# viswavi/speech-anonymization

Hardware: AMD Instinct MI355X
Metric: audio frames/sec (node), ConvAE+gender-adv train step (higher is better)
Workload: dtype bf16x3; 1 GPU; ConvAE recon0.1+sex0.9 adversarial train step (L1 recon + NLL), shape M: 32 utt/GPU x 161120 samples (T=1008 frames), Fbank x2 + norm + fwd + bwd + clip + Adam + Noam; batch_per_gpu=32, frames_per_utt=1008, parallelism=dp1

## Files before the change

### speech-anonymization_amd/csrc/sa_common.h

```cpp
#pragma once
#include <hip/hip_runtime.h>
#include <stdint.h>
#include "../../include/sa_hip.h"

typedef __bf16 bf16_t;
typedef __bf16 bf16x8 __attribute__((ext_vector_type(8)));
typedef float f32x16 __attribute__((ext_vector_type(16)));
typedef float f32x4 __attribute__((ext_vector_type(4)));

#define SA_WAVE 64


template <typename T> struct Tr;

template <> struct Tr<float> {
  static constexpr int VEC = 4;
  static constexpr int KS = 2;
  typedef float Frag;
  __device__ static inline void unpack(const uint4& u, float* f) {
    f[0] = __uint_as_float(u.x); f[1] = __uint_as_float(u.y);
    f[2] = __uint_as_float(u.z); f[3] = __uint_as_float(u.w);
  }
  __device__ static inline uint4 pack(const float* f) {
    return make_uint4(__float_as_uint(f[0]), __float_as_uint(f[1]),
                      __float_as_uint(f[2]), __float_as_uint(f[3]));
  }
  __device__ static inline float to_f(float v) { return v; }
  __device__ static inline float from_f(float v) { return v; }
  __device__ static inline f32x16 mfma(Frag a, Frag b, f32x16 c) {
    return __builtin_amdgcn_mfma_f32_32x32x2f32(a, b, c, 0, 0, 0);
  }
};

__device__ static inline uint32_t sa_pack_bf16x2(float lo, float hi) {
  union { bf16_t b[2]; uint32_t u; } cv;
  cv.b[0] = (bf16_t)lo; cv.b[1] = (bf16_t)hi;
  return cv.u;
}

template <> struct Tr<bf16_t> {
  static constexpr int VEC = 8;
  static constexpr int KS = 16;
  typedef bf16x8 Frag;
  __device__ static inline void unpack(const uint4& u, float* f) {
    f[0] = __uint_as_float(u.x << 16); f[1] = __uint_as_float(u.x & 0xffff0000u);
    f[2] = __uint_as_float(u.y << 16); f[3] = __uint_as_float(u.y & 0xffff0000u);
    f[4] = __uint_as_float(u.z << 16); f[5] = __uint_as_float(u.z & 0xffff0000u);
    f[6] = __uint_as_float(u.w << 16); f[7] = __uint_as_float(u.w & 0xffff0000u);
  }
  __device__ static inline uint4 pack(const float* f) {
    return make_uint4(sa_pack_bf16x2(f[0], f[1]), sa_pack_bf16x2(f[2], f[3]),
                      sa_pack_bf16x2(f[4], f[5]), sa_pack_bf16x2(f[6], f[7]));
  }
  __device__ static inline float to_f(bf16_t v) { return (float)v; }
  __device__ static inline bf16_t from_f(float v) { return (bf16_t)v; }
  __device__ static inline f32x16 mfma(Frag a, Frag b, f32x16 c) {
    return __builtin_amdgcn_mfma_f32_32x32x16_bf16(a, b, c, 0, 0, 0);
  }
};

__device__ static inline float sa_swish(float v) { return v * __builtin_amdgcn_rcpf(1.0f + __expf(-v)); }
__device__ static inline float sa_swish_grad(float v) {
  const float s = __builtin_amdgcn_rcpf(1.0f + __builtin_amdgcn_exp2f(v * -1.4426950408889634f));
  const float t = 1.0f - s;
  const float u = fmaf(v, t, 1.0f);
  return s * u;
}

__device__ static inline int sa_acc_row(int reg, int lane) {
  return (reg & 3) + 8 * (reg >> 2) + 4 * (lane >> 5);
}

__device__ static inline float sa_wave_sum(float v) {
#pragma unroll
  for (int o = 32; o > 0; o >>= 1) v += __shfl_xor(v, o, 64);
  return v;
}
__device__ static inline double sa_wave_sum_d(double v) {
#pragma unroll
  for (int o = 32; o > 0; o >>= 1) v += __shfl_xor(v, o, 64);
  return v;
}
__device__ static inline float sa_wave_max(float v) {
#pragma unroll
  for (int o = 32; o > 0; o >>= 1) v = fmaxf(v, __shfl_xor(v, o, 64));
  return v;
}

static inline int sa_div_up(int a, int b) { return (a + b - 1) / b; }

struct bf16x3_t {};
struct bf16x1f_t {};

struct fp8_t {};
typedef long fp8x8;

template <typename T> struct Pol;
template <> struct Pol<float> {
  typedef float store_t; typedef float lds_t; typedef float Frag;
  static constexpr int NPL = 1, VEC = 4, KS = 2, PAD = 1;
};
template <> struct Pol<bf16_t> {
  typedef bf16_t store_t; typedef bf16_t lds_t; typedef bf16x8 Frag;
  static constexpr int NPL = 1, VEC = 8, KS = 16, PAD = 8;
};
template <> struct Pol<bf16x1f_t> {
  typedef float store_t; typedef bf16_t lds_t; typedef bf16x8 Frag;
  static constexpr int NPL = 1, VEC = 4, KS = 16, PAD = 8;
};
template <> struct Pol<bf16x3_t> {
  typedef float store_t; typedef bf16_t lds_t; typedef bf16x8 Frag;
  static constexpr int NPL = 2, VEC = 4, KS = 16, PAD = 8;
};

template <> struct Pol<fp8_t> {
  typedef bf16_t store_t; typedef unsigned char lds_t; typedef fp8x8 Frag;
  static constexpr int NPL = 1, VEC = 8, KS = 16, PAD = 8;
};
template <> struct Tr<unsigned char> {
  __device__ static inline f32x16 mfma(fp8x8 a, fp8x8 b, f32x16 c) {
    return __builtin_amdgcn_mfma_f32_32x32x16_fp8_fp8(a, b, c, 0, 0, 0);
  }
};
__device__ static inline uint2 sa_pack_fp8x8(const float* f) {
  float c[8];
#pragma unroll
  for (int j = 0; j < 8; ++j) c[j] = __builtin_amdgcn_fmed3f(f[j], -448.0f, 448.0f);
  int lo = 0, hi = 0;
  lo = __builtin_amdgcn_cvt_pk_fp8_f32(c[0], c[1], lo, false);
  lo = __builtin_amdgcn_cvt_pk_fp8_f32(c[2], c[3], lo, true);
  hi = __builtin_amdgcn_cvt_pk_fp8_f32(c[4], c[5], hi, false);
  hi = __builtin_amdgcn_cvt_pk_fp8_f32(c[6], c[7], hi, true);
  return make_uint2((unsigned)lo, (unsigned)hi);
}

__device__ static inline uint2 sa_pack_bf16x4(const float* f) {
  return make_uint2(sa_pack_bf16x2(f[0], f[1]), sa_pack_bf16x2(f[2], f[3]));
}
__device__ static inline void sa_split4(const float* f, uint2& hi, uint2& lo) {
  float h[4], l[4];
#pragma unroll
  for (int j = 0; j < 4; ++j) {
    const bf16_t hb = (bf16_t)f[j];
    h[j] = (float)hb;
    l[j] = f[j] - h[j];
  }
  hi = sa_pack_bf16x4(h);
  lo = sa_pack_bf16x4(l);
}
```

### speech-anonymization_amd/csrc/sa_head.hip

```cpp
#include "sa_common.h"

template <typename T>
__global__ __launch_bounds__(256) void sa_pool_fwd_kernel(const T* __restrict__ r,
                                                          const float* __restrict__ sc,
                                                          const float* __restrict__ sh,
                                                          float* __restrict__ part, int L,
                                                          int nseg) {
  constexpr int C = 128, VEC = Tr<T>::VEC, CH = C / VEC, RPB = 256 / CH, NG = 128 / RPB;
  __shared__ float tile[RPB][C][2];
  const int tid = threadIdx.x, b = blockIdx.y, grp = blockIdx.x % NG, seg = blockIdx.x / NG;
  const int c = tid % CH, rl = tid / CH, lm = grp * RPB + rl;
  float s[VEC], t[VEC], sum[VEC], sq[VEC];
#pragma unroll
  for (int j = 0; j < VEC; ++j) { s[j] = sc[c * VEC + j]; t[j] = sh[c * VEC + j]; sum[j] = 0.f; sq[j] = 0.f; }
  const int nk = (L + 127) / 128, per = (nk + nseg - 1) / nseg;
  const int kbeg = seg * per, kend = (kbeg + per < nk) ? kbeg + per : nk;
  const T* rb = r + (size_t)b * L * C + c * VEC;
  for (int k0 = kbeg; k0 < kend; k0 += 4) {
    uint4 raw[4];
#pragma unroll
    for (int i = 0; i < 4; ++i) {
      const int l = lm + 128 * (k0 + i);
      raw[i] = make_uint4(0, 0, 0, 0);
      if (k0 + i < kend && l < L) raw[i] = *reinterpret_cast<const uint4*>(rb + (size_t)l * C);
    }
#pragma unroll
    for (int i = 0; i < 4; ++i) {
      const int l = lm + 128 * (k0 + i);
      if (k0 + i < kend && l < L) {
        float f[VEC];
        Tr<T>::unpack(raw[i], f);
#pragma unroll
        for (int j = 0; j < VEC; ++j) {
          const float v = fmaf(f[j], s[j], t[j]);
          sum[j] += v; sq[j] = fmaf(v, v, sq[j]);
        }
      }
    }
  }
#pragma unroll
  for (int j = 0; j < VEC; ++j) { tile[rl][c * VEC + j][0] = sum[j]; tile[rl][c * VEC + j][1] = sq[j]; }
  __syncthreads();
  float* dst = part + ((size_t)b * nseg + seg) * C * 128 * 2;
  for (int e = tid; e < RPB * C * 2; e += 256) {
    const int cc = e / (RPB * 2), w = e % (RPB * 2);
    dst[((size_t)cc * 128 + grp * RPB) * 2 + w] = tile[w >> 1][cc][w & 1];
  }
}

__global__ __launch_bounds__(1024) void sa_pool_gather_kernel(const float* __restrict__ part, int nseg,
                                                              int L, double* __restrict__ sums) {
  __shared__ double grp[7][128][2];
  const int tid = threadIdx.x, b = blockIdx.x, j = tid & 127, h = tid >> 7, Lm = L % 128;
  double s = 0.0, q = 0.0;
  for (int seg = 0; seg < nseg; ++seg) {
    const float2* p = reinterpret_cast<const float2*>(part) + ((size_t)b * nseg + seg) * 128 * 128;
#pragma unroll 16
    for (int c = h * 16; c < h * 16 + 16; ++c) {
      const float2 v = p[(size_t)c * 128 + ((j - c * Lm) & 127)];
      s += v.x; q += v.y;
    }
  }
  if (h > 0) { grp[h - 1][j][0] = s; grp[h - 1][j][1] = q; }
  __syncthreads();
  if (h == 0) {
#pragma unroll
    for (int g = 0; g < 7; ++g) { s += grp[g][j][0]; q += grp[g][j][1]; }
    sums[((size_t)b * 128 + j) * 2 + 0] = s;
    sums[((size_t)b * 128 + j) * 2 + 1] = q;
  }
}

extern "C" int sa_pool_nseg(int B) {
  int n = 2048 / (B * 16);
  return n < 1 ? 1 : (n > 8 ? 8 : n);
}

extern "C" int sa_pool_fwd(int dtype, const void* r, const float* scale, const float* shift,
                           float* part, int B, int L, int nseg, void* stream) {
  if (!r || !scale || !shift || !part || B <= 0 || L <= 1 || nseg < 1) return -22;
  hipStream_t st = reinterpret_cast<hipStream_t>(stream);
  if (dtype == SA_BF16)
    hipLaunchKernelGGL(sa_pool_fwd_kernel<bf16_t>, dim3(8 * nseg, B), dim3(256), 0, st,
                       reinterpret_cast<const bf16_t*>(r), scale, shift, part, L, nseg);
  else
    hipLaunchKernelGGL(sa_pool_fwd_kernel<float>, dim3(16 * nseg, B), dim3(256), 0, st,
                       reinterpret_cast<const float*>(r), scale, shift, part, L, nseg);
  hipError_t e = hipGetLastError();
  return e == hipSuccess ? 0 : -(int)e;
}

extern "C" int sa_pool_gather(const float* part, int B, int nseg, int L, double* sums, void* stream) {
  if (!part || !sums || B <= 0 || nseg < 1) return -22;
  hipLaunchKernelGGL(sa_pool_gather_kernel, dim3(B), dim3(1024), 0,
                     reinterpret_cast<hipStream_t>(stream), part, nseg, L, sums);
  hipError_t e = hipGetLastError();
  return e == hipSuccess ? 0 : -(int)e;
}

__global__ void sa_pool_fin_kernel(const double* __restrict__ sums, int B, int n,
                                   const float* __restrict__ noise, float eps, float* pooled,
                                   float* mean, float* stdraw) {
  const int i = blockIdx.x * blockDim.x + threadIdx.x;
  if (i >= B * 128) return;
  const int b = i / 128, j = i % 128;
  const double S = sums[2 * i], Q = sums[2 * i + 1];
  const double m = S / n;
  double var = (Q - S * m) / (n - 1);
  if (var < 0.0) var = 0.0;
  const float sd = (float)sqrt(var);
  mean[i] = (float)m; stdraw[i] = sd;
  float mo = (float)m;
  if (noise) mo += eps * ((1.0f - 9.0f) * noise[i] + 9.0f);
  pooled[(size_t)b * 256 + j] = mo;
  pooled[(size_t)b * 256 + 128 + j] = sd + eps;
}

extern "C" int sa_pool_fin(const double* sums, int B, int n, const float* noise, float eps,
                           float* pooled, float* mean, float* stdraw, void* stream) {
  if (!sums || !pooled || !mean || !stdraw || n < 2) return -22;
  hipLaunchKernelGGL(sa_pool_fin_kernel, dim3(sa_div_up(B * 128, 256)), dim3(256), 0,
                     reinterpret_cast<hipStream_t>(stream), sums, B, n, noise, eps, pooled, mean,
                     stdraw);
  hipError_t e = hipGetLastError();
  return e == hipSuccess ? 0 : -(int)e;
}

template <typename T>
__global__ __launch_bounds__(256) void sa_pool_bwd_kernel(const T* __restrict__ r,
                                                          const float* __restrict__ sc,
                                                          const float* __restrict__ sh,
                                                          const float* __restrict__ dpooled,
                                                          const float* __restrict__ mean,
                                                          const float* __restrict__ stdraw,
                                                          T* __restrict__ g, int L,
                                                          const float* __restrict__ bn_mean,
                                                          const float* __restrict__ bn_rstd,
                                                          float* __restrict__ stats) {
  constexpr int C = 128, VEC = Tr<T>::VEC, CH = C / VEC, RPP = 256 / CH;
  __shared__ float ka[128], kb[128];
  __shared__ float red[RPP][C][2];
  const int tid = threadIdx.x, b = blockIdx.y, l0 = blockIdx.x * SA_WAVE * 4;
  if (tid < 128) {
    const float dm = dpooled[(size_t)b * 256 + tid], ds = dpooled[(size_t)b * 256 + 128 + tid];
    const float sd = stdraw[(size_t)b * 128 + tid], m = mean[(size_t)b * 128 + tid];
    const float inv = sd > 0.0f ? 1.0f / ((float)(L - 1) * sd) : 0.0f;
    kb[tid] = ds * inv;
    ka[tid] = dm / (float)L - ds * inv * m;
  }
  __syncthreads();
  const int c = tid % CH, r0 = tid / CH;
  float s[VEC], t[VEC];
  int jb[VEC];
#pragma unroll
  for (int j = 0; j < VEC; ++j) {
    s[j] = sc[c * VEC + j]; t[j] = sh[c * VEC + j];
    jb[j] = (int)(((long long)(c * VEC + j) * L) % 128);
  }
  float bm[VEC], br[VEC], s1[VEC], s2[VEC];
#pragma unroll
  for (int j = 0; j < VEC; ++j) {
    bm[j] = stats ? bn_mean[c * VEC + j] : 0.0f;
    br[j] = stats ? bn_rstd[c * VEC + j] : 0.0f;
    s1[j] = 0.0f; s2[j] = 0.0f;
  }
  for (int rr = r0; rr < 256; rr += RPP) {
    const int l = l0 + rr;
    if (l >= L) break;
    float f[VEC], x[VEC];
    Tr<T>::unpack(*reinterpret_cast<const uint4*>(r + ((size_t)b * L + l) * C + c * VEC), x);
#pragma unroll
    for (int j = 0; j < VEC; ++j) {
      const int col = (jb[j] + l) % 128;
      f[j] = fmaf(kb[col], fmaf(x[j], s[j], t[j]), ka[col]);
    }
    const uint4 u = Tr<T>::pack(f);
    *reinterpret_cast<uint4*>(g + ((size_t)b * L + l) * C + c * VEC) = u;
    if (stats) {
      Tr<T>::unpack(u, f);
#pragma unroll
      for (int j = 0; j < VEC; ++j) {
        s1[j] += f[j];
        s2[j] = fmaf(f[j], (x[j] - bm[j]) * br[j], s2[j]);
      }
    }
  }
  if (stats) {
#pragma unroll
    for (int j = 0; j < VEC; ++j) { red[r0][c * VEC + j][0] = s1[j]; red[r0][c * VEC + j][1] = s2[j]; }
    __syncthreads();
    if (tid < C) {
      float a0 = 0.0f, a1 = 0.0f;
#pragma unroll
      for (int q = 0; q < RPP; ++q) { a0 += red[q][tid][0]; a1 += red[q][tid][1]; }
      float* dst = stats + (((size_t)b * gridDim.x + blockIdx.x) * C + tid) * 2;
      dst[0] = a0; dst[1] = a1;
    }
  }
}

extern "C" int sa_pool_bwd(int dtype, const void* r, const float* scale, const float* shift,
                           const float* dpooled, const float* mean, const float* stdraw, void* g,
                           int B, int L, const float* bn_mean, const float* bn_rstd, float* stats,
                           void* stream) {
  if (!r || !scale || !shift || !dpooled || !mean || !stdraw || !g || L < 2) return -22;
  if (stats && (!bn_mean || !bn_rstd)) return -22;
  hipStream_t st = reinterpret_cast<hipStream_t>(stream);
  dim3 grid(sa_div_up(L, 256), B);
  if (dtype == SA_BF16)
    hipLaunchKernelGGL(sa_pool_bwd_kernel<bf16_t>, grid, dim3(256), 0, st,
                       reinterpret_cast<const bf16_t*>(r), scale, shift, dpooled, mean, stdraw,
                       reinterpret_cast<bf16_t*>(g), L, bn_mean, bn_rstd, stats);
  else
    hipLaunchKernelGGL(sa_pool_bwd_kernel<float>, grid, dim3(256), 0, st,
                       reinterpret_cast<const float*>(r), scale, shift, dpooled, mean, stdraw,
                       reinterpret_cast<float*>(g), L, bn_mean, bn_rstd, stats);
  hipError_t e = hipGetLastError();
  return e == hipSuccess ? 0 : -(int)e;
}

__global__ __launch_bounds__(256) void sa_dense_kernel(const float* __restrict__ X, int lda,
                                                       const float* __restrict__ ps,
                                                       const float* __restrict__ pt,
                                                       const float* __restrict__ W, int sbk, int sbn,
                                                       const float* __restrict__ bias, float* __restrict__ Y,
                                                       int ldy, int M, int N, int K, int relu) {
  __shared__ float part[4][16][64];
  const int lane = threadIdx.x & 63, wave = threadIdx.x >> 6, n0 = blockIdx.x * 32, m0 = blockIdx.y * 32;
  const int m = m0 + (lane & 31), n = n0 + (lane & 31), kh = lane >> 5;
  f32x16 acc;
#pragma unroll
  for (int i = 0; i < 16; ++i) acc[i] = 0.0f;
  for (int k0 = wave * 16; k0 < K; k0 += 64) {
    float av[8], bv[8];
#pragma unroll
    for (int u = 0; u < 8; ++u) {
      const int k = k0 + 2 * u + kh;
      av[u] = 0.0f; bv[u] = 0.0f;
      if (k < K) {
        if (m < M) {
          av[u] = X[(size_t)m * lda + k];
          if (ps) av[u] = fmaf(av[u], ps[k], pt[k]);
        }
        if (n < N) bv[u] = W[(size_t)k * sbk + (size_t)n * sbn];
      }
    }
#pragma unroll
    for (int u = 0; u < 8; ++u)
      if (k0 + 2 * u < K) acc = __builtin_amdgcn_mfma_f32_32x32x2f32(av[u], bv[u], acc, 0, 0, 0);
  }
#pragma unroll
  for (int i = 0; i < 16; ++i) part[wave][i][lane] = acc[i];
  __syncthreads();
  if (wave == 0 && n < N) {
    const float bb = bias ? bias[n] : 0.0f;
#pragma unroll
    for (int i = 0; i < 16; ++i) {
      const int mr = m0 + sa_acc_row(i, lane);
      if (mr < M) {
        float v = ((part[0][i][lane] + part[1][i][lane]) + part[2][i][lane]) + part[3][i][lane] + bb;
        if (relu) v = fmaxf(v, 0.0f);
        Y[(size_t)mr * ldy + n] = v;
      }
    }
  }
}

extern "C" int sa_dense(const float* X, int lda, const float* ps, const float* pt, const float* W,
                        int sbk, int sbn, const float* bias, float* Y, int ldy, int M, int N, int K,
                        int relu, void* stream) {
  if (!X || !W || !Y || M <= 0 || N <= 0 || K <= 0) return -22;
  dim3 grid(sa_div_up(N, 32), sa_div_up(M, 32));
  hipLaunchKernelGGL(sa_dense_kernel, grid, dim3(256), 0, reinterpret_cast<hipStream_t>(stream), X,
                     lda, ps, pt, W, sbk, sbn, bias, Y, ldy, M, N, K, relu);
  hipError_t e = hipGetLastError();
  return e == hipSuccess ? 0 : -(int)e;
}

__global__ void sa_colsums_kernel(const float* __restrict__ X, const float* __restrict__ H,
                                  const float* __restrict__ hm, const float* __restrict__ hr,
                                  int M, int N, double* sums, float* __restrict__ out0,
                                  float* __restrict__ out1) {
  const int n = blockIdx.x * blockDim.x + threadIdx.x;
  if (n >= N) return;
  double s = 0.0, q = 0.0;
#pragma unroll 8
  for (int m = 0; m < M; ++m) {
    const float x = X[(size_t)m * N + n];
    float h = H ? H[(size_t)m * N + n] : x;
    if (hm) h = (h - hm[n]) * hr[n];
    s += x; q += (double)x * h;
  }
  sums[2 * n] = s; sums[2 * n + 1] = q;
  if (out0) out0[n] = (float)s;
  if (out1) out1[n] = (float)q;
}

extern "C" int sa_colsums(const float* X, const float* H, const float* hmean, const float* hrstd,
                          int M, int N, double* sums, float* out0, float* out1, void* stream) {
  if (!X || !sums) return -22;
  hipLaunchKernelGGL(sa_colsums_kernel, dim3(sa_div_up(N, 64)), dim3(64), 0,
                     reinterpret_cast<hipStream_t>(stream), X, H, hmean, hrstd, M, N, sums, out0,
                     out1);
  hipError_t e = hipGetLastError();
  return e == hipSuccess ? 0 : -(int)e;
}

__global__ void sa_bn2d_bwd_kernel(const float* __restrict__ G, const float* __restrict__ H,
                                   const double* __restrict__ sums, double count,
                                   const float* __restrict__ gamma, const float* __restrict__ mean,
                                   const float* __restrict__ rstd, int relu_mask, int M, int N,
                                   float* dH, const double* __restrict__ count_dev) {
  const int i = blockIdx.x * blockDim.x + threadIdx.x;
  if (i >= M * N) return;
  if (count_dev) count = *count_dev;
  const int n = i % N;
  const float hh = (H[i] - mean[n]) * rstd[n];
  float v = gamma[n] * rstd[n] * (G[i] - (float)(sums[2 * n] / count) - hh * (float)(sums[2 * n + 1] / count));
  if (relu_mask && !(H[i] > 0.0f)) v = 0.0f;
  dH[i] = v;
}

extern "C" int sa_bn2d_bwd(const float* G, const float* H, const double* sums, double count,
                           const float* gamma, const float* mean, const float* rstd, int relu_mask,
                           int M, int N, float* dH, const double* count_dev, void* stream) {
  if (!G || !H || !sums || !gamma || !mean || !rstd || !dH) return -22;
  hipLaunchKernelGGL(sa_bn2d_bwd_kernel, dim3(sa_div_up(M * N, 256)), dim3(256), 0,
                     reinterpret_cast<hipStream_t>(stream), G, H, sums, count, gamma, mean, rstd,
                     relu_mask, M, N, dH, count_dev);
  hipError_t e = hipGetLastError();
  return e == hipSuccess ? 0 : -(int)e;
}

__global__ void sa_dense_wgrad_kernel(const float* __restrict__ dY, const float* __restrict__ X,
                                      const float* __restrict__ ps, const float* __restrict__ pt,
                                      int M, int N, int K, float* dW) {
  const int i = blockIdx.x * blockDim.x + threadIdx.x;
  if (i >= N * K) return;
  const int n = i / K, k = i % K;
  float s = 0.0f;
#pragma unroll 8
  for (int m = 0; m < M; ++m) {
    float x = X[(size_t)m * K + k];
    if (ps) x = fmaf(x, ps[k], pt[k]);
    s = fmaf(dY[(size_t)m * N + n], x, s);
  }
  dW[i] = s;
}

extern "C" int sa_dense_wgrad(const float* dY, const float* X, const float* ps, const float* pt,
                              int M, int N, int K, float* dW, void* stream) {
  if (!dY || !X || !dW) return -22;
  hipLaunchKernelGGL(sa_dense_wgrad_kernel, dim3(sa_div_up(N * K, 256)), dim3(256), 0,
                     reinterpret_cast<hipStream_t>(stream), dY, X, ps, pt, M, N, K, dW);
  hipError_t e = hipGetLastError();
  return e == hipSuccess ? 0 : -(int)e;
}

__global__ void sa_log_softmax_kernel(const float* __restrict__ X, float* __restrict__ Y, int M, int N) {
  const int m = blockIdx.x * blockDim.x + threadIdx.x;
  if (m >= M) return;
  float mx = -INFINITY;
  for (int n = 0; n < N; ++n) mx = fmaxf(mx, X[(size_t)m * N + n]);
  float s = 0.0f;
  for (int n = 0; n < N; ++n) s += expf(X[(size_t)m * N + n] - mx);
  const float lse = mx + logf(s);
  for (int n = 0; n < N; ++n) Y[(size_t)m * N + n] = X[(size_t)m * N + n] - lse;
}
__global__ void sa_log_softmax_bwd_kernel(const float* __restrict__ dY, const float* __restrict__ Y,
                                          float* __restrict__ dX, int M, int N) {
  const int m = blockIdx.x * blockDim.x + threadIdx.x;
  if (m >= M) return;
  float s = 0.0f;
  for (int n = 0; n < N; ++n) s += dY[(size_t)m * N + n];
  for (int n = 0; n < N; ++n) dX[(size_t)m * N + n] = dY[(size_t)m * N + n] - expf(Y[(size_t)m * N + n]) * s;
}
extern "C" int sa_log_softmax(const float* X, float* Y, int M, int N, void* stream) {
  if (!X || !Y) return -22;
  hipLaunchKernelGGL(sa_log_softmax_kernel, dim3(sa_div_up(M, 64)), dim3(64), 0,
                     reinterpret_cast<hipStream_t>(stream), X, Y, M, N);
  hipError_t e = hipGetLastError();
  return e == hipSuccess ? 0 : -(int)e;
}
extern "C" int sa_log_softmax_bwd(const float* dY, const float* Y, float* dX, int M, int N, void* stream) {
  if (!dY || !Y || !dX) return -22;
  hipLaunchKernelGGL(sa_log_softmax_bwd_kernel, dim3(sa_div_up(M, 64)), dim3(64), 0,
                     reinterpret_cast<hipStream_t>(stream), dY, Y, dX, M, N);
  hipError_t e = hipGetLastError();
  return e == hipSuccess ? 0 : -(int)e;
}
// ... 138 lines not shown
```

### speech-anonymization_amd/csrc/sa_small.hip

```cpp
#include "sa_common.h"

#define SA_K15 15
#define SA_C32 32

template <typename T>
__global__ __launch_bounds__(256) void sa_conv1toC_kernel(const float* __restrict__ x,
                                                          const float* __restrict__ w,
                                                          const float* __restrict__ bias,
                                                          T* __restrict__ y, int L, int flip,
                                                          float* __restrict__ stats, int ntiles,
                                                          const T* __restrict__ ep_x,
                                                          const float* __restrict__ ep_s1,
                                                          const float* __restrict__ ep_t1,
                                                          const float* __restrict__ ep_mean,
                                                          const float* __restrict__ ep_rstd) {
  constexpr int VEC = Tr<T>::VEC, CH = SA_C32 / VEC, PPP = 256 / CH, TILE = 512;
  __shared__ float xs[TILE + SA_K15 - 1];
  __shared__ __attribute__((aligned(16))) float ws[SA_K15][SA_C32];
  __shared__ float red[PPP][SA_C32][2];
  const int tid = threadIdx.x, b = blockIdx.y, l0 = blockIdx.x * TILE;
  for (int i = tid; i < TILE + SA_K15 - 1; i += 256) {
    const int g = l0 + i - 7;
    xs[i] = (g >= 0 && g < L) ? x[(size_t)b * L + g] : 0.0f;
  }
  for (int i = tid; i < SA_K15 * SA_C32; i += 256) {
    const int k = i / SA_C32, c = i % SA_C32;
    ws[k][c] = w[c * SA_K15 + (flip ? SA_K15 - 1 - k : k)];
  }
  __syncthreads();
  const int c = tid % CH, p0 = tid / CH;
  float bv[VEC], ssum[VEC], ssq[VEC];
#pragma unroll
  for (int j = 0; j < VEC; ++j) { bv[j] = bias ? bias[c * VEC + j] : 0.0f; ssum[j] = 0.f; ssq[j] = 0.f; }
  float es[VEC], et[VEC], em[VEC], er[VEC];
#pragma unroll
  for (int j = 0; j < VEC; ++j) {
    const size_t bc = (size_t)b * SA_C32 + c * VEC + j;
    es[j] = ep_x ? ep_s1[bc] : 1.0f; et[j] = ep_x ? ep_t1[bc] : 0.0f;
    em[j] = ep_x ? ep_mean[bc] : 0.0f; er[j] = ep_x ? ep_rstd[bc] : 0.0f;
  }
  for (int p = p0; p < TILE; p += PPP) {
    const int l = l0 + p;
    if (l >= L) break;
    float acc[VEC];
#pragma unroll
    for (int j = 0; j < VEC; ++j) acc[j] = bv[j];
#pragma unroll
    for (int k = 0; k < SA_K15; ++k) {
      const float xv = xs[p + k];
#pragma unroll
      for (int j = 0; j < VEC; ++j) acc[j] = fmaf(xv, ws[k][c * VEC + j], acc[j]);
    }
    float xn[VEC];
    if (ep_x) {
      float xv[VEC];
      Tr<T>::unpack(*reinterpret_cast<const uint4*>(ep_x + ((size_t)b * L + l) * SA_C32 + c * VEC), xv);
#pragma unroll
      for (int j = 0; j < VEC; ++j) {
        acc[j] *= sa_swish_grad(fmaf(xv[j], es[j], et[j]));
        xn[j] = (xv[j] - em[j]) * er[j];
      }
    }
    const uint4 u = Tr<T>::pack(acc);
    *reinterpret_cast<uint4*>(y + ((size_t)b * L + l) * SA_C32 + c * VEC) = u;
    if (stats) {
      float f[VEC];
      Tr<T>::unpack(u, f);
#pragma unroll
      for (int j = 0; j < VEC; ++j) { ssum[j] += f[j]; ssq[j] = fmaf(f[j], ep_x ? xn[j] : f[j], ssq[j]); }
    }
  }
  if (stats) {
#pragma unroll
    for (int j = 0; j < VEC; ++j) { red[p0][c * VEC + j][0] = ssum[j]; red[p0][c * VEC + j][1] = ssq[j]; }
    __syncthreads();
    if (tid < SA_C32) {
      float s = 0.f, q = 0.f;
      for (int r = 0; r < PPP; ++r) { s += red[r][tid][0]; q += red[r][tid][1]; }
      float* d = stats + (((size_t)b * ntiles + blockIdx.x) * SA_C32 + tid) * 2;
      d[0] = s; d[1] = q;
    }
  }
}

extern "C" int sa_conv1toC_ntiles(int L) { return sa_div_up(L, 512); }

extern "C" int sa_conv1toC(int dtype, const float* x, const float* w, const float* bias, void* y,
                           int B, int L, int flip, float* stats, const void* ep_x, const float* ep_s1,
                           const float* ep_t1, const float* ep_mean, const float* ep_rstd,
                           void* stream) {
  if (!x || !w || !y || B <= 0 || L <= 0) return -22;
  if (ep_x && (!ep_s1 || !ep_t1 || !ep_mean || !ep_rstd)) return -22;
  hipStream_t st = reinterpret_cast<hipStream_t>(stream);
  const int nt = sa_div_up(L, 512);
  dim3 grid(nt, B);
  if (dtype == SA_BF16)
    hipLaunchKernelGGL(sa_conv1toC_kernel<bf16_t>, grid, dim3(256), 0, st, x, w, bias,
                       reinterpret_cast<bf16_t*>(y), L, flip, stats, nt,
                       reinterpret_cast<const bf16_t*>(ep_x), ep_s1, ep_t1, ep_mean, ep_rstd);
  else
    hipLaunchKernelGGL(sa_conv1toC_kernel<float>, grid, dim3(256), 0, st, x, w, bias,
                       reinterpret_cast<float*>(y), L, flip, stats, nt,
                       reinterpret_cast<const float*>(ep_x), ep_s1, ep_t1, ep_mean, ep_rstd);
  hipError_t e = hipGetLastError();
  return e == hipSuccess ? 0 : -(int)e;
}

template <typename T>
__global__ __launch_bounds__(256) void sa_convCto1_kernel(const T* __restrict__ x,
                                                          const float* __restrict__ w,
                                                          const float* __restrict__ bias,
                                                          float* __restrict__ y, int L,
                                                          const float* __restrict__ s1,
                                                          const float* __restrict__ t1, int swish,
                                                          int flip) {
  constexpr int VEC = Tr<T>::VEC, CH = SA_C32 / VEC, RPP = 256 / CH, TILE = 128, PITCH = 36;
  constexpr int NPOS = TILE + SA_K15 - 1, NBLK = (NPOS + 15) / 16, TP = 17;
  constexpr int NIT = (NBLK * 16 + RPP - 1) / RPP;
  __shared__ __attribute__((aligned(16))) float xs[NBLK * 16 * PITCH];
  __shared__ float tp[NBLK * 16 * TP];
  const int tid = threadIdx.x, lane = tid & 63, wave = tid >> 6, b = blockIdx.y, l0 = blockIdx.x * TILE;
  {
    const int c = tid % CH, r0 = tid / CH;
    float sc[VEC], sh[VEC];
#pragma unroll
    for (int j = 0; j < VEC; ++j) {
      sc[j] = s1 ? s1[(size_t)b * SA_C32 + c * VEC + j] : 1.0f;
      sh[j] = t1 ? t1[(size_t)b * SA_C32 + c * VEC + j] : 0.0f;
    }
    uint4 raw[NIT];
#pragma unroll
    for (int i = 0; i < NIT; ++i) {
      const int r = r0 + i * RPP, g = l0 + r - 7;
      raw[i] = make_uint4(0, 0, 0, 0);
      if (r < NPOS && g >= 0 && g < L)
        raw[i] = *reinterpret_cast<const uint4*>(x + ((size_t)b * L + g) * SA_C32 + c * VEC);
    }
#pragma unroll
    for (int i = 0; i < NIT; ++i) {
      const int r = r0 + i * RPP, g = l0 + r - 7;
      if (r < NBLK * 16) {
        float f[VEC];
        Tr<T>::unpack(raw[i], f);
        const bool valid = r < NPOS && g >= 0 && g < L;
#pragma unroll
        for (int j = 0; j < VEC; ++j) {
          float v = fmaf(f[j], sc[j], sh[j]);
          v = swish ? sa_swish(v) : v;
          xs[r * PITCH + c * VEC + j] = valid ? v : 0.0f;
        }
      }
    }
  }
  const int n = lane & 15, kq = lane >> 4;
  float wb[8];
#pragma unroll
  for (int ks = 0; ks < 8; ++ks)
    wb[ks] = n < SA_K15 ? w[(ks * 4 + kq) * SA_K15 + (flip ? SA_K15 - 1 - n : n)] : 0.0f;
  __syncthreads();
  for (int blk = wave; blk < NBLK; blk += 4) {
    f32x4 acc = {0.f, 0.f, 0.f, 0.f};
    const float* ap = xs + (blk * 16 + n) * PITCH + kq;
#pragma unroll
    for (int ks = 0; ks < 8; ++ks) acc = __builtin_amdgcn_mfma_f32_16x16x4f32(ap[ks * 4], wb[ks], acc, 0, 0, 0);
#pragma unroll
    for (int i = 0; i < 4; ++i) tp[(blk * 16 + 4 * kq + i) * TP + n] = acc[i];
  }
  __syncthreads();
  const int l = l0 + tid;
  if (tid < TILE && l < L) {
    float acc = bias ? bias[0] : 0.0f;
#pragma unroll
    for (int k = 0; k < SA_K15; ++k) acc += tp[(tid + k) * TP + k];
    y[(size_t)b * L + l] = acc;
  }
}

extern "C" int sa_convCto1(int dtype, const void* x, const float* w, const float* bias, float* y,
                           int B, int L, const float* s1, const float* t1, int swish, int flip,
                           void* stream) {
  if (!x || !w || !y || B <= 0 || L <= 0) return -22;
  hipStream_t st = reinterpret_cast<hipStream_t>(stream);
  dim3 grid(sa_div_up(L, 128), B);
  if (dtype == SA_BF16)
    hipLaunchKernelGGL(sa_convCto1_kernel<bf16_t>, grid, dim3(256), 0, st,
                       reinterpret_cast<const bf16_t*>(x), w, bias, y, L, s1, t1, swish, flip);
  else
    hipLaunchKernelGGL(sa_convCto1_kernel<float>, grid, dim3(256), 0, st,
                       reinterpret_cast<const float*>(x), w, bias, y, L, s1, t1, swish, flip);
  hipError_t e = hipGetLastError();
  return e == hipSuccess ? 0 : -(int)e;
}

template <typename T>
__global__ __launch_bounds__(256) void sa_wgrad1C_kernel(const float* __restrict__ u,
                                                         const T* __restrict__ v,
                                                         float* __restrict__ slabs, int L,
                                                         int chunk, int flip,
                                                         const float* __restrict__ s1,
                                                         const float* __restrict__ t1, int swish) {
  constexpr int VEC = Tr<T>::VEC, CH = SA_C32 / VEC, RPP = 256 / CH, TILE = 256, PITCH = 33;
  __shared__ float us[TILE + SA_K15 - 1 + 1];
  __shared__ float vs[TILE * PITCH];
  const int tid = threadIdx.x, lane = tid & 63, wave = tid >> 6, b = blockIdx.y;
  const int lbeg = blockIdx.x * chunk;
  int lend = lbeg + chunk; if (lend > L) lend = L;
  const int c = tid % CH, r0 = tid / CH;
  float sc[VEC], sh[VEC];
#pragma unroll
  for (int j = 0; j < VEC; ++j) {
    sc[j] = s1 ? s1[(size_t)b * SA_C32 + c * VEC + j] : 1.0f;
    sh[j] = t1 ? t1[(size_t)b * SA_C32 + c * VEC + j] : 0.0f;
  }
  const bool tr_on = (s1 != nullptr) || swish;
  const int m = lane & 15, j4 = lane >> 4;
  const bool mval = m < SA_K15;
  const int kk = mval ? (flip ? SA_K15 - 1 - m : m) : 0;
  const int qa = wave * 64 + 16 * j4;
  f32x4 acc0 = {0.f, 0.f, 0.f, 0.f}, acc1 = {0.f, 0.f, 0.f, 0.f};
  constexpr int NIT = TILE / RPP, NU = (TILE + SA_K15 - 1 + 255) / 256;
  uint4 raw[NIT];
  float rawu[NU];
  auto issue = [&](int l0) {
#pragma unroll
    for (int i = 0; i < NIT; ++i) {
      const int g = l0 + r0 + i * RPP;
      raw[i] = make_uint4(0, 0, 0, 0);
      if (g < lend) raw[i] = *reinterpret_cast<const uint4*>(v + ((size_t)b * L + g) * SA_C32 + c * VEC);
    }
#pragma unroll
    for (int i = 0; i < NU; ++i) {
      const int g = l0 + tid + i * 256 - 7;
      rawu[i] = (l0 < lend && tid + i * 256 < TILE + SA_K15 - 1 && g >= 0 && g < L) ? u[(size_t)b * L + g] : 0.0f;
    }
  };
  issue(lbeg);
  for (int l0 = lbeg; l0 < lend; l0 += TILE) {
#pragma unroll
    for (int i = 0; i < NU; ++i)
      if (tid + i * 256 < TILE + SA_K15 - 1) us[tid + i * 256] = rawu[i];
#pragma unroll
    for (int i = 0; i < NIT; ++i) {
      const int r = r0 + i * RPP, g = l0 + r;
      float f[VEC];
      Tr<T>::unpack(raw[i], f);
      if (tr_on && g < lend) {
#pragma unroll
        for (int j = 0; j < VEC; ++j) {
          float z = fmaf(f[j], sc[j], sh[j]);
          f[j] = swish ? sa_swish(z) : z;
        }
      }
#pragma unroll
      for (int j = 0; j < VEC; ++j) vs[r * PITCH + c * VEC + j] = f[j];
    }
    __syncthreads();
    issue(l0 + TILE);
#pragma unroll 4
    for (int t = 0; t < 16; ++t) {
      const int q = qa + t;
      const float av = mval ? us[q + kk] : 0.0f;
      const float b0 = vs[q * PITCH + m], b1 = vs[q * PITCH + 16 + m];
      acc0 = __builtin_amdgcn_mfma_f32_16x16x4f32(av, b0, acc0, 0, 0, 0);
      acc1 = __builtin_amdgcn_mfma_f32_16x16x4f32(av, b1, acc1, 0, 0, 0);
    }
    __syncthreads();
  }
  float* part = vs;
#pragma unroll
  for (int i = 0; i < 4; ++i) {
    part[(wave * 16 + 4 * j4 + i) * 32 + m] = acc0[i];
    part[(wave * 16 + 4 * j4 + i) * 32 + 16 + m] = acc1[i];
  }
  __syncthreads();
  for (int o = tid; o < SA_K15 * SA_C32; o += 256) {
    const int k = o / SA_C32, cc = o % SA_C32;
    const float sum = ((part[(0 * 16 + k) * 32 + cc] + part[(1 * 16 + k) * 32 + cc]) +
                       part[(2 * 16 + k) * 32 + cc]) + part[(3 * 16 + k) * 32 + cc];
    slabs[((size_t)b * gridDim.x + blockIdx.x) * (SA_C32 * SA_K15) + cc * SA_K15 + k] = sum;
  }
}

extern "C" int sa_wgrad1C_nchunk(int L, int chunk) { return sa_div_up(L, chunk); }

extern "C" int sa_wgrad1C(int dtype, const float* u, const void* v, float* slabs, int B, int L,
                          int chunk, int flip, const float* s1, const float* t1, int swish,
                          void* stream) {
  if (!u || !v || !slabs || B <= 0 || L <= 0 || chunk <= 0 || chunk % 256) return -22;
  hipStream_t st = reinterpret_cast<hipStream_t>(stream);
  dim3 grid(sa_div_up(L, chunk), B);
  if (dtype == SA_BF16)
    hipLaunchKernelGGL(sa_wgrad1C_kernel<bf16_t>, grid, dim3(256), 0, st, u,
                       reinterpret_cast<const bf16_t*>(v), slabs, L, chunk, flip, s1, t1, swish);
  else
    hipLaunchKernelGGL(sa_wgrad1C_kernel<float>, grid, dim3(256), 0, st, u,
                       reinterpret_cast<const float*>(v), slabs, L, chunk, flip, s1, t1, swish);
  hipError_t e = hipGetLastError();
  return e == hipSuccess ? 0 : -(int)e;
}

template <typename T>
__global__ __launch_bounds__(256, Tr<T>::VEC == 4 ? 3 : 2) void sa_bwd1C_kernel(const float* __restrict__ u,
                                                       const T* __restrict__ v,
                                                       const float* __restrict__ w,
                                                       T* __restrict__ gout, float* __restrict__ stats,
                                                       int ntiles, float* __restrict__ slabs, int L,
                                                       int chunk, int flip,
                                                       const float* __restrict__ s1,
                                                       const float* __restrict__ t1,
                                                       const float* __restrict__ mean,
                                                       const float* __restrict__ rstd) {
  constexpr int VEC = Tr<T>::VEC, CH = SA_C32 / VEC, RPP = 256 / CH, TILE = 256, PITCH = 33;
  __shared__ float us[TILE + SA_K15 - 1 + 1];
  __shared__ float vs[TILE * PITCH];
  __shared__ __attribute__((aligned(16))) float ws[SA_K15][SA_C32];
  __shared__ float red[RPP][SA_C32][2];
  __shared__ __attribute__((aligned(16))) float pv[4][SA_C32];
  const int tid = threadIdx.x, lane = tid & 63, wave = tid >> 6, b = blockIdx.y;
  const int lbeg = blockIdx.x * chunk;
  int lend = lbeg + chunk; if (lend > L) lend = L;
  const int c = tid % CH, r0 = tid / CH;
  float ssum[VEC], ssq[VEC];
#pragma unroll
  for (int j = 0; j < VEC; ++j) { ssum[j] = 0.f; ssq[j] = 0.f; }
  if (tid < 4 * SA_C32) {
    const float* src = tid < 32 ? s1 : tid < 64 ? t1 : tid < 96 ? mean : rstd;
    pv[tid >> 5][tid & 31] = src[(size_t)b * SA_C32 + (tid & 31)];
  }
  for (int i = tid; i < SA_K15 * SA_C32; i += 256) {
    const int k = i / SA_C32, cc = i % SA_C32;
    ws[k][cc] = w[cc * SA_K15 + (flip ? SA_K15 - 1 - k : k)];
  }
  const int m = lane & 15, j4 = lane >> 4;
  const bool mval = m < SA_K15;
  const int kk = mval ? (flip ? SA_K15 - 1 - m : m) : 0;
  const int qa = wave * 64 + 16 * j4;
  f32x4 acc0 = {0.f, 0.f, 0.f, 0.f}, acc1 = {0.f, 0.f, 0.f, 0.f};
  constexpr int NIT = TILE / RPP, NU = (TILE + SA_K15 - 1 + 255) / 256;
  uint4 raw[NIT];
  float rawu[NU];
  auto issue_v = [&](int l0, int i) {
    const int g = l0 + r0 + i * RPP;
    raw[i] = make_uint4(0, 0, 0, 0);
    if (g < lend) raw[i] = *reinterpret_cast<const uint4*>(v + ((size_t)b * L + g) * SA_C32 + c * VEC);
  };
  auto issue_u = [&](int l0) {
#pragma unroll
    for (int i = 0; i < NU; ++i) {
      const int g = l0 + tid + i * 256 - 7;
      rawu[i] = (l0 < lend && tid + i * 256 < TILE + SA_K15 - 1 && g >= 0 && g < L) ? u[(size_t)b * L + g] : 0.0f;
    }
  };
#pragma unroll
  for (int i = 0; i < NIT; ++i) issue_v(lbeg, i);
  issue_u(lbeg);
  __syncthreads();
  for (int l0 = lbeg; l0 < lend; l0 += TILE) {
#pragma unroll
    for (int i = 0; i < NU; ++i)
      if (tid + i * 256 < TILE + SA_K15 - 1) us[tid + i * 256] = rawu[i];
#pragma unroll
    for (int i = 0; i < NIT; ++i) {
      const int r = r0 + i * RPP, g = l0 + r;
      float f[VEC];
      Tr<T>::unpack(raw[i], f);
      if (g < lend) {
        int z0 = c * VEC; asm volatile("" : "+v"(z0));
#pragma unroll
        for (int j = 0; j < VEC; ++j) f[j] = sa_swish(fmaf(f[j], pv[0][z0 + j], pv[1][z0 + j]));
      }
#pragma unroll
      for (int j = 0; j < VEC; ++j) vs[r * PITCH + c * VEC + j] = f[j];
    }
    __syncthreads();
    issue_u(l0 + TILE);
#pragma unroll
    for (int i = 0; i < NIT; ++i) {
      const int r = r0 + i * RPP, g = l0 + r;
      float xv[VEC];
      Tr<T>::unpack(raw[i], xv);
      issue_v(l0 + TILE, i);
      if (g < lend) {
#pragma clang fp contract(off)
        float acc[VEC], xn[VEC];
#pragma unroll
        for (int j = 0; j < VEC; ++j) acc[j] = 0.0f;
#pragma unroll
        for (int k = 0; k < SA_K15; ++k) {
          const float uv = us[r + k];
#pragma unroll
          for (int j = 0; j < VEC; ++j) acc[j] = fmaf(uv, ws[k][c * VEC + j], acc[j]);
        }
        int z0 = c * VEC; asm volatile("" : "+v"(z0));
#pragma unroll
        for (int j = 0; j < VEC; ++j) {
          acc[j] *= sa_swish_grad(fmaf(xv[j], pv[0][z0 + j], pv[1][z0 + j]));
          xn[j] = (xv[j] - pv[2][z0 + j]) * pv[3][z0 + j];
        }
        const uint4 o = Tr<T>::pack(acc);
        *reinterpret_cast<uint4*>(gout + ((size_t)b * L + g) * SA_C32 + c * VEC) = o;
        float f[VEC];
        Tr<T>::unpack(o, f);
#pragma unroll
        for (int j = 0; j < VEC; ++j) { ssum[j] += f[j]; ssq[j] = fmaf(f[j], xn[j], ssq[j]); }
      }
    }
    const bool flush = (((l0 - lbeg) / TILE) & 1) || l0 + TILE >= lend;
    if (flush) {
#pragma unroll
      for (int j = 0; j < VEC; ++j) {
        red[r0][c * VEC + j][0] = ssum[j]; red[r0][c * VEC + j][1] = ssq[j];
        ssum[j] = 0.f; ssq[j] = 0.f;
      }
    }
#pragma unroll 4
    for (int t = 0; t < 16; ++t) {
      const int q = qa + t;
      const float av = mval ? us[q + kk] : 0.0f;
      const float b0 = vs[q * PITCH + m], b1 = vs[q * PITCH + 16 + m];
      acc0 = __builtin_amdgcn_mfma_f32_16x16x4f32(av, b0, acc0, 0, 0, 0);
      acc1 = __builtin_amdgcn_mfma_f32_16x16x4f32(av, b1, acc1, 0, 0, 0);
    }
    __syncthreads();
    if (flush && tid < SA_C32) {
      float s = 0.f, q = 0.f;
      for (int r = 0; r < RPP; ++r) { s += red[r][tid][0]; q += red[r][tid][1]; }
      float* d = stats + (((size_t)b * ntiles + l0 / 512) * SA_C32 + tid) * 2;
      d[0] = s; d[1] = q;
    }
  }
  float* part = vs;
#pragma unroll
  for (int i = 0; i < 4; ++i) {
    part[(wave * 16 + 4 * j4 + i) * 32 + m] = acc0[i];
    part[(wave * 16 + 4 * j4 + i) * 32 + 16 + m] = acc1[i];
  }
  __syncthreads();
  for (int o = tid; o < SA_K15 * SA_C32; o += 256) {
    const int k = o / SA_C32, cc = o % SA_C32;
    const float sum = ((part[(0 * 16 + k) * 32 + cc] + part[(1 * 16 + k) * 32 + cc]) +
                       part[(2 * 16 + k) * 32 + cc]) + part[(3 * 16 + k) * 32 + cc];
    slabs[((size_t)b * gridDim.x + blockIdx.x) * (SA_C32 * SA_K15) + cc * SA_K15 + k] = sum;
  }
}

extern "C" int sa_bwd1C(int dtype, const float* u, const void* v, const float* w, void* g, float* stats,
                        float* slabs, int B, int L, int chunk, int flip, const float* s1,
                        const float* t1, const float* mean, const float* rstd, void* stream) {
  if (!u || !v || !w || !g || !stats || !slabs || B <= 0 || L <= 0 || chunk <= 0 || chunk % 512) return -22;
  if (!s1 || !t1 || !mean || !rstd) return -22;
  hipStream_t st = reinterpret_cast<hipStream_t>(stream);
  const int nt = sa_div_up(L, 512);
  dim3 grid(sa_div_up(L, chunk), B);
  if (dtype == SA_BF16)
    hipLaunchKernelGGL(sa_bwd1C_kernel<bf16_t>, grid, dim3(256), 0, st, u,
                       reinterpret_cast<const bf16_t*>(v), w, reinterpret_cast<bf16_t*>(g), stats, nt,
                       slabs, L, chunk, flip, s1, t1, mean, rstd);
  else
    hipLaunchKernelGGL(sa_bwd1C_kernel<float>, grid, dim3(256), 0, st, u,
                       reinterpret_cast<const float*>(v), w, reinterpret_cast<float*>(g), stats, nt,
                       slabs, L, chunk, flip, s1, t1, mean, rstd);
  hipError_t e = hipGetLastError();
  return e == hipSuccess ? 0 : -(int)e;
}

__global__ __launch_bounds__(256) void sa_sum_slabs_kernel(const float* __restrict__ slabs,
                                                           float* __restrict__ dst, int nslab, int n,
                                                           int accumulate) {
  __shared__ double part[16][17];
  const int o = threadIdx.x & 15, q = threadIdx.x >> 4, i = blockIdx.x * 16 + o;
  double s = 0.0;
  if (i < n) {
#pragma unroll 4
    for (int k = q; k < nslab; k += 16) s += (double)slabs[(size_t)k * n + i];
  }
  part[q][o] = s;
  __syncthreads();
  if (q == 0 && i < n) {
    double t = 0.0;
#pragma unroll
    for (int r = 0; r < 16; ++r) t += part[r][o];
    dst[i] = accumulate ? dst[i] + (float)t : (float)t;
  }
}

extern "C" int sa_sum_slabs(const float* slabs, float* dst, int nslab, int n, int accumulate,
                            void* stream) {
  if (!slabs || !dst || nslab <= 0 || n <= 0) return -22;
  hipLaunchKernelGGL(sa_sum_slabs_kernel, dim3(sa_div_up(n, 16)), dim3(256), 0,
                     reinterpret_cast<hipStream_t>(stream), slabs, dst, nslab, n, accumulate);
  hipError_t e = hipGetLastError();
  return e == hipSuccess ? 0 : -(int)e;
}
```

Before: 3.942 million frames/s.

## Add tile-walking conv1toC/convCto1 kernels and nontemporal loads for streamed activations

Adds persistent-style walk kernels for the 1-to-C and C-to-1 convolutions. Each workgroup now walks several tiles with double-buffered input prefetch, replacing one workgroup per tile. The C-to-1 conv is rebuilt around small f32 MFMAs plus a shifted-sum reduction through LDS. Separately, the pooling and weight-gradient kernels switch their streamed activation reads to nontemporal loads. All new paths are on by default, with SA_STREAM_V1=1 restoring the old kernels; the cost is fewer, longer-running workgroups and more code paths to keep correct.

Result: no change. 3.975 million frames/s, median of 6 (+0.8%).

```diff
diff --git a/speech-anonymization_amd/csrc/sa_common.h b/speech-anonymization_amd/csrc/sa_common.h
--- a/speech-anonymization_amd/csrc/sa_common.h
+++ b/speech-anonymization_amd/csrc/sa_common.h
@@ -1,6 +1,7 @@
 #pragma once
 #include <hip/hip_runtime.h>
 #include <stdint.h>
+#include <stdlib.h>
 #include "../../include/sa_hip.h"
 
 typedef __bf16 bf16_t;
@@ -58,6 +59,19 @@
     return __builtin_amdgcn_mfma_f32_32x32x16_bf16(a, b, c, 0, 0, 0);
   }
 };
+
+typedef uint32_t sa_u32x4 __attribute__((ext_vector_type(4)));
+template <bool NT> __device__ static inline uint4 sa_ld16(const void* p) {
+  if (NT) {
+    const sa_u32x4 v = __builtin_nontemporal_load(reinterpret_cast<const sa_u32x4*>(p));
+    return make_uint4(v.x, v.y, v.z, v.w);
+  }
+  return *reinterpret_cast<const uint4*>(p);
+}
+static inline bool sa_stream_v1() {
+  const char* e = getenv("SA_STREAM_V1");
+  return e && e[0] == '1' && e[1] == 0;
+}
 
 __device__ static inline float sa_swish(float v) { return v * __builtin_amdgcn_rcpf(1.0f + __expf(-v)); }
 __device__ static inline float sa_swish_grad(float v) {
diff --git a/speech-anonymization_amd/csrc/sa_head.hip b/speech-anonymization_amd/csrc/sa_head.hip
--- a/speech-anonymization_amd/csrc/sa_head.hip
+++ b/speech-anonymization_amd/csrc/sa_head.hip
@@ -1,6 +1,6 @@
 #include "sa_common.h"
 
-template <typename T>
+template <typename T, bool NT>
 __global__ __launch_bounds__(256) void sa_pool_fwd_kernel(const T* __restrict__ r,
                                                           const float* __restrict__ sc,
                                                           const float* __restrict__ sh,
@@ -22,7 +22,7 @@
     for (int i = 0; i < 4; ++i) {
       const int l = lm + 128 * (k0 + i);
       raw[i] = make_uint4(0, 0, 0, 0);
-      if (k0 + i < kend && l < L) raw[i] = *reinterpret_cast<const uint4*>(rb + (size_t)l * C);
+      if (k0 + i < kend && l < L) raw[i] = sa_ld16<NT>(rb + (size_t)l * C);
     }
 #pragma unroll
     for (int i = 0; i < 4; ++i) {
@@ -80,12 +80,13 @@
                            float* part, int B, int L, int nseg, void* stream) {
   if (!r || !scale || !shift || !part || B <= 0 || L <= 1 || nseg < 1) return -22;
   hipStream_t st = reinterpret_cast<hipStream_t>(stream);
-  if (dtype == SA_BF16)
-    hipLaunchKernelGGL(sa_pool_fwd_kernel<bf16_t>, dim3(8 * nseg, B), dim3(256), 0, st,
-                       reinterpret_cast<const bf16_t*>(r), scale, shift, part, L, nseg);
-  else
-    hipLaunchKernelGGL(sa_pool_fwd_kernel<float>, dim3(16 * nseg, B), dim3(256), 0, st,
-                       reinterpret_cast<const float*>(r), scale, shift, part, L, nseg);
+  const bool nt = !sa_stream_v1();
+#define SA_POOL_FWD(T, NT, NGRP)                                                                   \
+  hipLaunchKernelGGL((sa_pool_fwd_kernel<T, NT>), dim3(NGRP * nseg, B), dim3(256), 0, st,            \
+                     reinterpret_cast<const T*>(r), scale, shift, part, L, nseg)
+  if (dtype == SA_BF16) { if (nt) SA_POOL_FWD(bf16_t, true, 8); else SA_POOL_FWD(bf16_t, false, 8); }
+  else { if (nt) SA_POOL_FWD(float, true, 16); else SA_POOL_FWD(float, false, 16); }
+#undef SA_POOL_FWD
   hipError_t e = hipGetLastError();
   return e == hipSuccess ? 0 : -(int)e;
 }
diff --git a/speech-anonymization_amd/csrc/sa_small.hip b/speech-anonymization_amd/csrc/sa_small.hip
--- a/speech-anonymization_amd/csrc/sa_small.hip
+++ b/speech-anonymization_amd/csrc/sa_small.hip
@@ -83,6 +83,104 @@
   }
 }
 
+template <typename T, bool EP>
+__global__ __launch_bounds__(256, Tr<T>::VEC == 4 ? (EP ? 3 : 4) : 2)
+void sa_conv1toC_walk_kernel(const float* __restrict__ x, const float* __restrict__ w,
+                             const float* __restrict__ bias, T* __restrict__ y, int L, int flip,
+                             float* __restrict__ stats, int ntiles, int tpw, const T* __restrict__ ep_x,
+                             const float* __restrict__ ep_s1, const float* __restrict__ ep_t1,
+                             const float* __restrict__ ep_mean, const float* __restrict__ ep_rstd) {
+  constexpr int VEC = Tr<T>::VEC, CH = SA_C32 / VEC, PPP = 256 / CH, TILE = 512;
+  constexpr int NX = TILE + SA_K15 - 1, NU = (NX + 255) / 256;
+  __shared__ float xs[2][NX + 2];
+  __shared__ float red[2][PPP][SA_C32][2];
+  const int tid = threadIdx.x, b = blockIdx.y;
+  const int t0 = blockIdx.x * tpw;
+  int t1 = t0 + tpw; if (t1 > ntiles) t1 = ntiles;
+  const int c = tid % CH, p0 = tid / CH;
+  float rawx[NU];
+  auto issue_x = [&](int t) {
+#pragma unroll
+    for (int i = 0; i < NU; ++i) {
+      const int g = t * TILE + tid + i * 256 - 7;
+      rawx[i] = (t < t1 && tid + i * 256 < NX && g >= 0 && g < L) ? x[(size_t)b * L + g] : 0.0f;
+    }
+  };
+  auto put_x = [&](int buf) {
+#pragma unroll
+    for (int i = 0; i < NU; ++i)
+      if (tid + i * 256 < NX) xs[buf][tid + i * 256] = rawx[i];
+  };
+  issue_x(t0);
+  float wr[SA_K15][VEC], bv[VEC];
+#pragma unroll
+  for (int k = 0; k < SA_K15; ++k)
+#pragma unroll
+    for (int j = 0; j < VEC; ++j) wr[k][j] = w[(c * VEC + j) * SA_K15 + (flip ? SA_K15 - 1 - k : k)];
+#pragma unroll
+  for (int j = 0; j < VEC; ++j) bv[j] = bias ? bias[c * VEC + j] : 0.0f;
+  float es[VEC], et[VEC], em[VEC], er[VEC];
+#pragma unroll
+  for (int j = 0; j < VEC; ++j) {
+    const size_t bc = (size_t)b * SA_C32 + c * VEC + j;
+    es[j] = EP ? ep_s1[bc] : 1.0f; et[j] = EP ? ep_t1[bc] : 0.0f;
+    em[j] = EP ? ep_mean[bc] : 0.0f; er[j] = EP ? ep_rstd[bc] : 0.0f;
+  }
+  put_x(t0 & 1);
+  __syncthreads();
+  for (int t = t0; t < t1; ++t) {
+    const int l0 = t * TILE, cur = t & 1;
+    issue_x(t + 1);
+    float ssum[VEC], ssq[VEC];
+#pragma unroll
+    for (int j = 0; j < VEC; ++j) { ssum[j] = 0.f; ssq[j] = 0.f; }
+    for (int p = p0; p < TILE; p += PPP) {
+#pragma clang fp contract(off)
+      const int l = l0 + p;
+      if (l >= L) break;
+      float acc[VEC];
+#pragma unroll
+      for (int j = 0; j < VEC; ++j) acc[j] = bv[j];
+#pragma unroll
+      for (int k = 0; k < SA_K15; ++k) {
+        const float xv = xs[cur][p + k];
+#pragma unroll
+        for (int j = 0; j < VEC; ++j) acc[j] = fmaf(xv, wr[k][j], acc[j]);
+      }
+      float xn[VEC];
+      if (EP) {
+        float xv[VEC];
+        Tr<T>::unpack(*reinterpret_cast<const uint4*>(ep_x + ((size_t)b * L + l) * SA_C32 + c * VEC), xv);
+#pragma unroll
+        for (int j = 0; j < VEC; ++j) {
+          acc[j] *= sa_swish_grad(fmaf(xv[j], es[j], et[j]));
+          xn[j] = (xv[j] - em[j]) * er[j];
+        }
+      }
+      const uint4 u = Tr<T>::pack(acc);
+      *reinterpret_cast<uint4*>(y + ((size_t)b * L + l) * SA_C32 + c * VEC) = u;
+      if (stats) {
+        float f[VEC];
+        Tr<T>::unpack(u, f);
+#pragma unroll
+        for (int j = 0; j < VEC; ++j) { ssum[j] += f[j]; ssq[j] = fmaf(f[j], EP ? xn[j] : f[j], ssq[j]); }
+      }
+    }
+    put_x(cur ^ 1);
+    if (stats) {
+#pragma unroll
+      for (int j = 0; j < VEC; ++j) { red[cur][p0][c * VEC + j][0] = ssum[j]; red[cur][p0][c * VEC + j][1] = ssq[j]; }
+    }
+    __syncthreads();
+    if (stats && tid < SA_C32) {
+      float s = 0.f, q = 0.f;
+      for (int r = 0; r < PPP; ++r) { s += red[cur][r][tid][0]; q += red[cur][r][tid][1]; }
+      float* d = stats + (((size_t)b * ntiles + t) * SA_C32 + tid) * 2;
+      d[0] = s; d[1] = q;
+    }
+  }
+}
+
 extern "C" int sa_conv1toC_ntiles(int L) { return sa_div_up(L, 512); }
 
 extern "C" int sa_conv1toC(int dtype, const float* x, const float* w, const float* bias, void* y,
@@ -93,6 +191,19 @@
   if (ep_x && (!ep_s1 || !ep_t1 || !ep_mean || !ep_rstd)) return -22;
   hipStream_t st = reinterpret_cast<hipStream_t>(stream);
   const int nt = sa_div_up(L, 512);
+  if (!sa_stream_v1()) {
+    const int tpw = 4;
+    dim3 wgrid(sa_div_up(nt, tpw), B);
+#define SA_WALK(T, EP)                                                                                  \
+  hipLaunchKernelGGL((sa_conv1toC_walk_kernel<T, EP>), wgrid, dim3(256), 0, st, x, w, bias,               \
+                     reinterpret_cast<T*>(y), L, flip, stats, nt, tpw, reinterpret_cast<const T*>(ep_x), \
+                     ep_s1, ep_t1, ep_mean, ep_rstd)
+    if (dtype == SA_BF16) { if (ep_x) SA_WALK(bf16_t, true); else SA_WALK(bf16_t, false); }
+    else { if (ep_x) SA_WALK(float, true); else SA_WALK(float, false); }
+#undef SA_WALK
+    hipError_t e = hipGetLastError();
+    return e == hipSuccess ? 0 : -(int)e;
+  }
   dim3 grid(nt, B);
   if (dtype == SA_BF16)
     hipLaunchKernelGGL(sa_conv1toC_kernel<bf16_t>, grid, dim3(256), 0, st, x, w, bias,
@@ -176,11 +287,100 @@
   }
 }
 
+template <typename T>
+__global__ __launch_bounds__(256) void sa_convCto1_walk_kernel(const T* __restrict__ x,
+                                                               const float* __restrict__ w,
+                                                               const float* __restrict__ bias,
+                                                               float* __restrict__ y, int L,
+                                                               const float* __restrict__ s1,
+                                                               const float* __restrict__ t1, int swish,
+                                                               int flip, int opw) {
+  constexpr int VEC = Tr<T>::VEC, CH = SA_C32 / VEC, RPP = 256 / CH, STEP = 128, PITCH = 36, TP = 17;
+  constexpr int NIT = STEP / RPP;
+  __shared__ __attribute__((aligned(16))) float xs[STEP * PITCH];
+  __shared__ float tp[2 * STEP * TP];
+  const int tid = threadIdx.x, lane = tid & 63, wave = tid >> 6, b = blockIdx.y;
+  const int lbeg = blockIdx.x * opw;
+  const int nout = L - lbeg < opw ? L - lbeg : opw;
+  const int nsteps = (nout + SA_K15 - 1 + STEP - 1) / STEP;
+  const int c = tid % CH, r0 = tid / CH;
+  float sc[VEC], sh[VEC];
+#pragma unroll
+  for (int j = 0; j < VEC; ++j) {
+    sc[j] = s1 ? s1[(size_t)b * SA_C32 + c * VEC + j] : 1.0f;
+    sh[j] = t1 ? t1[(size_t)b * SA_C32 + c * VEC + j] : 0.0f;
+  }
+  uint4 raw[NIT];
+  auto issue = [&](int s) {
+#pragma unroll
+    for (int i = 0; i < NIT; ++i) {
+      const int g = lbeg - 7 + s * STEP + r0 + i * RPP;
+      raw[i] = make_uint4(0, 0, 0, 0);
+      if (s < nsteps && g >= 0 && g < L) raw[i] = sa_ld16<true>(x + ((size_t)b * L + g) * SA_C32 + c * VEC);
+    }
+  };
+  issue(0);
+  const int n = lane & 15, kq = lane >> 4;
+  float wb[8];
+#pragma unroll
+  for (int ks = 0; ks < 8; ++ks)
+    wb[ks] = n < SA_K15 ? w[(ks * 4 + kq) * SA_K15 + (flip ? SA_K15 - 1 - n : n)] : 0.0f;
+  const float bv = bias ? bias[0] : 0.0f;
+  for (int s = 0; s < nsteps; ++s) {
+#pragma unroll
+    for (int i = 0; i < NIT; ++i) {
+      const int r = r0 + i * RPP, g = lbeg - 7 + s * STEP + r;
+      float f[VEC];
+      Tr<T>::unpack(raw[i], f);
+      const bool valid = g >= 0 && g < L;
+#pragma unroll
+      for (int j = 0; j < VEC; ++j) {
+        float v = fmaf(f[j], sc[j], sh[j]);
+        v = swish ? sa_swish(v) : v;
+        xs[r * PITCH + c * VEC + j] = valid ? v : 0.0f;
+      }
+    }
+    __syncthreads();
+    issue(s + 1);
+    float* tph = tp + (s & 1) * STEP * TP;
+#pragma unroll
+    for (int bi = 0; bi < 2; ++bi) {
+      const int blk = wave * 2 + bi;
+      f32x4 acc = {0.f, 0.f, 0.f, 0.f};
+      const float* ap = xs + (blk * 16 + n) * PITCH + kq;
+#pragma unroll
+      for (int ks = 0; ks < 8; ++ks) acc = __builtin_amdgcn_mfma_f32_16x16x4f32(ap[ks * 4], wb[ks], acc, 0, 0, 0);
+#pragma unroll
+      for (int i = 0; i < 4; ++i) tph[(blk * 16 + 4 * kq + i) * TP + n] = acc[i];
+    }
+    __syncthreads();
+    const int o = s * STEP - (SA_K15 - 1) + tid;
+    if (tid < STEP && o >= 0 && o < nout) {
+      float acc = bv;
+#pragma unroll
+      for (int k = 0; k < SA_K15; ++k) acc += tp[((o + k) & (2 * STEP - 1)) * TP + k];
+      y[(size_t)b * L + lbeg + o] = acc;
+    }
+  }
+}
+
 extern "C" int sa_convCto1(int dtype, const void* x, const float* w, const float* bias, float* y,
                            int B, int L, const float* s1, const float* t1, int swish, int flip,
                            void* stream) {
   if (!x || !w || !y || B <= 0 || L <= 0) return -22;
   hipStream_t st = reinterpret_cast<hipStream_t>(stream);
+  if (!sa_stream_v1()) {
+    const int opw = 128 * 8 - (SA_K15 - 1);
+    dim3 wgrid(sa_div_up(L, opw), B);
+    if (dtype == SA_BF16)
+      hipLaunchKernelGGL(sa_convCto1_walk_kernel<bf16_t>, wgrid, dim3(256), 0, st,
+                         reinterpret_cast<const bf16_t*>(x), w, bias, y, L, s1, t1, swish, flip, opw);
+    else
+      hipLaunchKernelGGL(sa_convCto1_walk_kernel<float>, wgrid, dim3(256), 0, st,
+                         reinterpret_cast<const float*>(x), w, bias, y, L, s1, t1, swish, flip, opw);
+    hipError_t e = hipGetLastError();
+    return e == hipSuccess ? 0 : -(int)e;
+  }
   dim3 grid(sa_div_up(L, 128), B);
   if (dtype == SA_BF16)
     hipLaunchKernelGGL(sa_convCto1_kernel<bf16_t>, grid, dim3(256), 0, st,
@@ -192,7 +392,7 @@
   return e == hipSuccess ? 0 : -(int)e;
 }
 
-template <typename T>
+template <typename T, bool NT>
 __global__ __launch_bounds__(256) void sa_wgrad1C_kernel(const float* __restrict__ u,
                                                          const T* __restrict__ v,
                                                          float* __restrict__ slabs, int L,
@@ -226,7 +426,7 @@
     for (int i = 0; i < NIT; ++i) {
       const int g = l0 + r0 + i * RPP;
       raw[i] = make_uint4(0, 0, 0, 0);
-      if (g < lend) raw[i] = *reinterpret_cast<const uint4*>(v + ((size_t)b * L + g) * SA_C32 + c * VEC);
+      if (g < lend) raw[i] = sa_ld16<NT>(v + ((size_t)b * L + g) * SA_C32 + c * VEC);
     }
 #pragma unroll
     for (int i = 0; i < NU; ++i) {
@@ -289,12 +489,13 @@
   if (!u || !v || !slabs || B <= 0 || L <= 0 || chunk <= 0 || chunk % 256) return -22;
   hipStream_t st = reinterpret_cast<hipStream_t>(stream);
   dim3 grid(sa_div_up(L, chunk), B);
-  if (dtype == SA_BF16)
-    hipLaunchKernelGGL(sa_wgrad1C_kernel<bf16_t>, grid, dim3(256), 0, st, u,
-                       reinterpret_cast<const bf16_t*>(v), slabs, L, chunk, flip, s1, t1, swish);
-  else
-    hipLaunchKernelGGL(sa_wgrad1C_kernel<float>, grid, dim3(256), 0, st, u,
-                       reinterpret_cast<const float*>(v), slabs, L, chunk, flip, s1, t1, swish);
+#define SA_WGRAD1C(T, NT)                                                                   \
+  hipLaunchKernelGGL((sa_wgrad1C_kernel<T, NT>), grid, dim3(256), 0, st, u,                   \
+                     reinterpret_cast<const T*>(v), slabs, L, chunk, flip, s1, t1, swish)
+  const bool nt = !sa_stream_v1();
+  if (dtype == SA_BF16) { if (nt) SA_WGRAD1C(bf16_t, true); else SA_WGRAD1C(bf16_t, false); }
+  else { if (nt) SA_WGRAD1C(float, true); else SA_WGRAD1C(float, false); }
+#undef SA_WGRAD1C
   hipError_t e = hipGetLastError();
   return e == hipSuccess ? 0 : -(int)e;
 }
```
